# benedikthoward/ENPH459-Super-Resolution

Measured on AMD Instinct MI355X. Metric: HR megapixels/sec at x4 upscale (SAA + 80-iteration IBP reconstruction), higher is better.
Workload: dtype f32; 1 GPU; C2: x4 multi-frame SR of 64x64 LR patches -> 256x256 HR, N=16 frames (all 4x4 sub-pixel phases), 7x7 Gaussian PSF, shift_and_add + ibp(80 it, step 0.5); patches_per_gpu=1024, global_patches=1024, factor=4, frames=16, n_iter=80, parallelism=patch-sharded x1, no collective

## Files before the change

enph459-super-resolution_amd/csrc/srx_api.hip:

```cpp
#include <cstdio>
#include <cstring>

#include "srx_prims.hpp"
#include "srx_fused.hpp"
#include "srx_route.hpp"
#include "srx_btile.hpp"
#include "srx_metrics.hpp"
#include "srx_psf.hpp"
#include "srx_register.hpp"
#include "srx_mean.hpp"
#include "srx_png.hpp"
#include "srx_crc.hpp"
#include "srx_patches.hpp"

using namespace srx;

static thread_local const char *g_last_path = "none";

namespace srx {
Profiler &profiler()
{
    static Profiler p;
    return p;
}
// ... 643 lines not shown
int srx_ibp_plan_get_rows_f32(srx_plan_t *p, int row_lo, int row_hi, float *dst, srx_stream_t s) { return plan_rows<float>(p, row_lo, row_hi, dst, false, hs(s)); }
int srx_ibp_plan_set_rows_f32(srx_plan_t *p, int row_lo, int row_hi, const float *src, srx_stream_t s)
{
    return plan_rows<float>(p, row_lo, row_hi, const_cast<float *>(src), true, hs(s));
}
int srx_ibp_plan_get_rows_f64(srx_plan_t *p, int row_lo, int row_hi, double *dst, srx_stream_t s) { return plan_rows<double>(p, row_lo, row_hi, dst, false, hs(s)); }
int srx_ibp_plan_set_rows_f64(srx_plan_t *p, int row_lo, int row_hi, const double *src, srx_stream_t s)
{
    return plan_rows<double>(p, row_lo, row_hi, const_cast<double *>(src), true, hs(s));
}
const char *srx_ibp_plan_path(srx_plan_t *p) { return p ? p->path : "none"; }
int srx_ibp_plan_supports_trace_rows(srx_plan_t *p) { return p && p->z ? 1 : 0; }
void srx_ibp_plan_destroy(srx_plan_t *p) { delete p; }

int srx_version(void) { return 100; }

#ifdef SRX_STAMPS
int srx_debug_stamps(unsigned long long *host_out)
{
    if (hipDeviceSynchronize() != hipSuccess)
        return SRX_E_HIP;
    if (hipMemcpyFromSymbol(host_out, HIP_SYMBOL(srx::srx_dbg_stamps), sizeof(unsigned long long) * 5 * 8 * 40000) != hipSuccess)
        return SRX_E_HIP;
    return SRX_OK;
}
int srx_debug_pstamps(unsigned long long *host_out)
{
    if (hipDeviceSynchronize() != hipSuccess)
        return SRX_E_HIP;
    if (hipMemcpyFromSymbol(host_out, HIP_SYMBOL(srx::srx_dbg_pstamps), sizeof(unsigned long long) * 24 * 4096) != hipSuccess)
        return SRX_E_HIP;
    return SRX_OK;
}
#endif

const char *srx_strerror(int s)
{
    switch (s) {
    case SRX_OK: return "ok";
    case SRX_E_INVALID: return "invalid argument";
    case SRX_E_UNSUPPORTED: return "unsupported configuration";
    case SRX_E_WORKSPACE: return "workspace missing, not 256-byte aligned or too small";
    case SRX_E_HIP: return "HIP runtime error";
    default: return "unknown status";
    }
}

const char *srx_last_path(void) { return g_last_path; }

void srx_profile_enable(int on)
{
    profiler().clear();
    profiler().on = on != 0;
}

int srx_profile_kernel_count(void) { return KID_COUNT; }

const char *srx_profile_kernel_name(int id) { return id >= 0 && id < KID_COUNT ? g_kernel_names[id] : ""; }

int srx_profile_get(int id, double *total_ms, long *launches)
{
    if (id < 0 || id >= KID_COUNT || !total_ms || !launches)
        return SRX_E_INVALID;
    Profiler &pf = profiler();
    std::lock_guard<std::mutex> g(pf.mu);
    double tot = 0.0;
// ... 416 lines not shown
```

enph459-super-resolution_amd/csrc/srx_common.h:

```cpp
#pragma once
#include <hip/hip_runtime.h>
#include <stddef.h>
#include <stdint.h>
#include <stdlib.h>
#include <string.h>

#include <atomic>
#include <mutex>
#include <type_traits>
#include <vector>

#include "srx.h"

#define SRX_NPAD 12
#define SRX_HORIZON 64

namespace srx {

template <typename T> __host__ __device__ constexpr T pole() { return (T)-0.26794919243112270647; }

template <typename T> struct AxisTap {
    int idx[4];
    T w[4];
};
// ... 254 lines not shown
    const unsigned orig = blockIdx.x + gx * (blockIdx.y + gy * blockIdx.z);
    const unsigned xcd = orig & 7u, q = nwg >> 3, r = nwg & 7u;
    const unsigned id = (xcd < r ? xcd * (q + 1) : r * (q + 1) + (xcd - r) * q) + (orig >> 3);
    bx = (int)(id % gx);
    by = (int)((id / gx) % gy);
    bz = (int)(id / (gx * gy));
}

__device__ __forceinline__ unsigned xcd_index(unsigned orig, unsigned n)
{
    const unsigned xcd = orig & 7u, q = n >> 3, r = n & 7u;
    return (xcd < r ? xcd * (q + 1) : r * (q + 1) + (xcd - r) * q) + (orig >> 3);
}
__device__ __forceinline__ void xcd_block_2d(int &bx, int &by)
{
    const unsigned gx = gridDim.x, id = xcd_index(blockIdx.x + gx * blockIdx.y, gx * gridDim.y);
    bx = (int)(id % gx);
    by = (int)(id / gx);
}

#ifdef SRX_STAMPS
__device__ unsigned long long srx_dbg_stamps[5][8][40000];
#define SRX_STAMP(K, PH)                                                                                       \
    do {                                                                                                        \
        if (threadIdx.x == 0 && threadIdx.y == 0) {                                                             \
            unsigned long long _t;                                                                               \
            asm volatile("s_memtime %0\n\ts_waitcnt lgkmcnt(0)" : "=s"(_t)::"memory");                         \
            const unsigned _blk = blockIdx.x + gridDim.x * (blockIdx.y + gridDim.y * blockIdx.z);                \
            if (_blk < 40000)                                                                                    \
                srx_dbg_stamps[K][PH][_blk] = _t;                                                                \
        }                                                                                                       \
    } while (0)
__device__ unsigned long long srx_dbg_pstamps[24][4096];
#define SRX_PSTAMP(PH)                                                                                         \
    do {                                                                                                        \
        __builtin_amdgcn_sched_barrier(0);                                                                      \
        const unsigned _lb = blockIdx.x + gridDim.x * blockIdx.y;                                               \
        const unsigned _sl = _lb * (blockDim.x >> 6) + (threadIdx.x >> 6);                                      \
        if ((threadIdx.x & 63) == 0 && _sl < 4096 && blockIdx.z == 0) {                                         \
            unsigned long long _t;                                                                               \
            asm volatile("s_memtime %0\n\ts_waitcnt lgkmcnt(0)" : "=s"(_t)::"memory");                         \
            srx_dbg_pstamps[PH][_sl] = _t;                                                                       \
        }                                                                                                       \
        __builtin_amdgcn_sched_barrier(0);                                                                      \
    } while (0)
#else
#define SRX_STAMP(K, PH) do { } while (0)
#define SRX_PSTAMP(PH) do { } while (0)
#endif

__device__ __forceinline__ void err_trace_reduce(const double *__restrict__ epart, int nblk, int item, double base,
                                                 double *__restrict__ out, int tid, double *part4)
{
    const double *p = epart + (size_t)item * nblk;
    double acc[8];
#pragma unroll
    for (int u = 0; u < 8; u++)
        acc[u] = 0.0;
    for (int i = tid; i < nblk; i += 256 * 8) {
#pragma unroll
        for (int u = 0; u < 8; u++) {
            const int k = i + 256 * u;
            acc[u] += k < nblk ? p[k] : 0.0;
        }
    }
    double s = ((acc[0] + acc[1]) + (acc[2] + acc[3])) + ((acc[4] + acc[5]) + (acc[6] + acc[7]));
    s = wave_sum(s);
    if ((tid & 63) == 0)
        part4[tid >> 6] = s;
    __syncthreads();
    if (tid == 0)
        *out = base + ((part4[0] + part4[1]) + (part4[2] + part4[3]));
    __syncthreads();
}

__device__ __forceinline__ void bspline3_weights(double t, double w[4])
{
    double y = t, z = 1.0 - t;
    w[1] = (y * y * (y - 2.0) * 3.0 + 4.0) / 6.0;
    w[2] = (z * z * (z - 2.0) * 3.0 + 4.0) / 6.0;
    w[0] = z * z * z / 6.0;
// ... 5 lines not shown
```

enph459-super-resolution_amd/csrc/srx_mosaic.hpp:

```cpp
#pragma once
#include <algorithm>
#include <type_traits>

#include "srx_fused.hpp"

namespace srx {
namespace mosaic {

constexpr int FWD_BATCH = 24;
using fused::corr7_strip8;
using fused::Kernel7;
using fused::TileCfg;

struct AxisPlan {
    double delta;
    int zero, E, D, PB, RS;
    int n[SRX_MAX_FRAMES];
    int nmin, nmax;
};

struct AxisDev {
    int E, D;
    int n[SRX_MAX_FRAMES];
};

template <typename T> struct MosaicArgs {
    int Dy, Dx, PBy, PBx;
    int RSy, RSx;
    T wfy[4], wfx[4];
    T wby[4], wbx[4];
};

struct MTap {
    int i;
    int rho;
};

static inline bool plan_axis(int N, const double *sh, int axis, int f, AxisPlan &pl)
{
    for (int k = 0; k < N; k++) {
        const double d = sh[2 * k + axis] * f;
        double n = std::floor(d), fr = d - n;
        if (fr > 1.0 - 1e-12)
            n += 1.0, fr = 0.0;
        if (fr < 1e-12)
            fr = 0.0;
        if (k == 0)
            pl.delta = fr;
        else if (std::fabs(fr - pl.delta) > 1e-12)
            return false;
        pl.n[k] = (int)n;
    }
    pl.zero = pl.delta == 0.0;
    pl.E = pl.zero ? 11 : 10;
    pl.D = 13 - pl.E;
    pl.nmin = pl.nmax = pl.n[0];
    for (int k = 1; k < N; k++)
        pl.nmin = std::min(pl.nmin, pl.n[k]), pl.nmax = std::max(pl.nmax, pl.n[k]);
    pl.PB = 13 - pl.nmin;
    pl.RS = std::max(13 - pl.nmax, 0);
    return true;
}

static inline bool eligible(const IbpSpec &s)
{
    if (!fused::ibp_eligible(s) || s.f < 2)
        return false;
    AxisPlan a;
    return plan_axis(s.N, s.sh, 0, s.f, a) && plan_axis(s.N, s.sh, 1, s.f, a) && s.H >= 32 && s.W >= 32;
}

__global__ void __launch_bounds__(64) k_build_mtaps(MTap *__restrict__ tab, int len, int n_img, int f, AxisDev ax)
{
    const int p = blockIdx.x * 64 + threadIdx.x, k = blockIdx.y;
    if (p >= len)
        return;
    const int u = p + ax.n[k] - 13;
    MTap t;
    if (u < 0) {
        t.i = 0;
        t.rho = ax.E - ax.n[k];
    } else if (u <= n_img - 1 && u % f == 0) {
        t.i = u / f;
        t.rho = p - ax.D;
    } else {
        t.i = -1;
        t.rho = 0;
    }
    tab[(size_t)k * len + p] = t;
}

__device__ __forceinline__ int near_index(int p, int q, int Wg, int PBy, int PBx)
{
    return p < PBy ? p * Wg + q : PBy * Wg + (p - PBy) * PBx + q;
}

template <typename T, int IB, int PXT, typename S = T>
__global__ void __launch_bounds__(256)
    k_mosaic_build(const S *__restrict__ lr, int B, int N, int h, int w, const MTap *__restrict__ tabY,
                   const MTap *__restrict__ tabX, int Hg, int Wg, int PBy, int PBx, int Dy, int Dx, int NB,
                   T *__restrict__ Mg, T *__restrict__ Cg, T *__restrict__ Mu, double *__restrict__ Vpart, int tr_lo, int tr_hi)
{
    __shared__ double part[4][IB];
    const int q0 = blockIdx.x * 64 * PXT + threadIdx.x, p = blockIdx.y * 4 + threadIdx.y, b0 = blockIdx.z * IB;
    const int pu = __builtin_amdgcn_readfirstlane(p);
    const size_t item = (size_t)N * h * w;
    double var[IB];
#pragma unroll
    for (int i = 0; i < IB; i++)
        var[i] = 0.0;
    if (pu < Hg) {
        double M[PXT][IB], S1[PXT][IB], S2[PXT][IB];
        int C[PXT], Cu[PXT];
#pragma unroll
        for (int c = 0; c < PXT; c++) {
            C[c] = Cu[c] = 0;
#pragma unroll
            for (int i = 0; i < IB; i++)
                M[c][i] = S1[c][i] = S2[c][i] = 0.0;
        }
        for (int k = 0; k < N; k++) {
            const MTap ty = tabY[(size_t)k * Hg + pu];
// ... 943 lines not shown
{
    return {ar.take<T>(d.B * d.Hg * d.Wg), ar.take<T>(d.Hg * d.Wg), ar.take<T>(d.B * d.NB), ar.take<MTap>(d.N * d.ty), ar.take<MTap>(d.N * d.tx),
            ar.take<double>(d.B), ar.take<double>(d.B * cdiv((int)d.Wg, 64) * cdiv((int)d.Hg, 4)), ar.take<int>(d.NB), ar.take<int>(d.NB * d.NS)};
}
static inline size_t ws_common(const IbpShape &s, int B)
{
    const size_t Hg = s.H + 2 * SRX_NPAD + 3, Wg = s.W + 2 * SRX_NPAD + 3, tl = Hg > Wg ? Hg : Wg;
    const CommonDims d{(size_t)B, (size_t)s.N, Hg, Wg, tl, tl, near_bound(Hg, Wg), near_slots(s.N)};
    return measured([&](Arena &m) { s.eb == 8 ? (void)carve_common<double>(m, d) : (void)carve_common<float>(m, d); });
}

template <typename T, typename S = T>
static int common_prep(Common<T> &c, bool own_build, const IbpCall<T, S> &call, Arena &ar, int tr_lo, int tr_hi)
{
    const IbpSpec &s = call.s;
    const int B = call.B, N = s.N, h = s.h, w = s.w, H = s.H, W = s.W, f = s.f;
    const S *const lr = call.lr;
    const hipStream_t st = call.st;
    const int Hp = H + 2 * SRX_NPAD, Wp = W + 2 * SRX_NPAD, Hg = Hp + 3, Wg = Wp + 3;
    static_assert(std::is_same<S, T>::value || std::is_same<S, uint8_t>::value, "LR samples: T or uint8_t");
    c.lr = lr, c.lr_u8 = !std::is_same<S, T>::value, c.B = B, c.N = N, c.h = h, c.w = w, c.H = H, c.W = W, c.f = f, c.flags = s.flags, c.step = call.step;
    c.scale = 1.0 / ((double)h * (double)w) / (double)N;
    AxisPlan &py = c.py, &px = c.px;
    if (!plan_axis(N, s.sh, 0, f, py) || !plan_axis(N, s.sh, 1, f, px))
        return SRX_E_UNSUPPORTED;
    const int NB = py.PB * Wg + (Hg - py.PB) * px.PB;
    const int NS = (int)near_slots(N);
    c.NB = NB, c.NS = NS, c.Hg = Hg, c.Wg = Wg;
    const auto [Mg, Cg, Mu, tabY, tabX, Vtot, Vpart, ncu, nyx] =
        carve_common<T>(ar, CommonDims{(size_t)B, (size_t)N, (size_t)Hg, (size_t)Wg, (size_t)Hg, (size_t)Wg, (size_t)NB, (size_t)NS});
    if (!ar.ok)
        return SRX_E_WORKSPACE;
    c.Mg = Mg, c.Cg = Cg, c.Mu = Mu, c.tabY = tabY, c.tabX = tabX, c.Vtot = Vtot, c.ncu = ncu, c.nyx = nyx;
    AxisDev dy, dx;
    dy.E = py.E, dy.D = py.D, dx.E = px.E, dx.D = px.D;
    for (int q = 0; q < SRX_MAX_FRAMES; q++)
        dy.n[q] = q < N ? py.n[q] : 0, dx.n[q] = q < N ? px.n[q] : 0;
    MosaicArgs<T> &ma = c.ma;
    ma.Dy = py.D, ma.Dx = px.D, ma.PBy = py.PB, ma.PBx = px.PB, ma.RSy = py.RS, ma.RSx = px.RS;
    fused::axis_firs<T>(py.delta, px.delta, 1.0, ma.wfy, ma.wfx, ma.wby, ma.wbx);
    fused::make_kernel7<T>(s.k, s.kh, s.kw, false, c.kc, s.flags);
    fused::make_kernel7<T>(s.k, s.kh, s.kw, true, c.kt, s.flags);
    c.sep = c.kc.separable && c.kt.separable, c.zero = py.zero && px.zero;
    hipLaunchKernelGGL(k_build_mtaps, dim3(cdiv(Hg, 64), N), dim3(64), 0, st, tabY, Hg, H, f, dy);
    SRX_CHECK_LAUNCH();
    hipLaunchKernelGGL(k_build_mtaps, dim3(cdiv(Wg, 64), N), dim3(64), 0, st, tabX, Wg, W, f, dx);
    SRX_CHECK_LAUNCH();
    if (fill_bytes(Vtot, 0, (size_t)B * sizeof(double), st) != hipSuccess)
        return SRX_E_HIP;
    c.own_build = own_build;
    if (!own_build) {
        if (B >= 8)
            SRX_LAUNCH(KID_MOSAIC_BUILD, (k_mosaic_build<T, 8, 1, S>), dim3(cdiv(Wg, 64), cdiv(Hg, 4), cdiv(B, 8)), dim3(64, 4), 0, st, lr, B, N, h,
                       w, tabY, tabX, Hg, Wg, py.PB, px.PB, py.D, px.D, NB, Mg, Cg, Mu, Vpart, tr_lo, tr_hi);
        else
            SRX_LAUNCH(KID_MOSAIC_BUILD, (k_mosaic_build<T, 1, 4, S>), dim3(cdiv(Wg, 256), cdiv(Hg, 4), B), dim3(64, 4), 0, st, lr, B, N, h, w,
                       tabY, tabX, Hg, Wg, py.PB, px.PB, py.D, px.D, NB, Mg, Cg, Mu, Vpart, tr_lo, tr_hi);
        hipLaunchKernelGGL(k_vtot_reduce, dim3(B), dim3(256), 0, st, Vpart, (B >= 8 ? cdiv(Wg, 64) : cdiv(Wg, 256)) * cdiv(Hg, 4), Vtot);
        SRX_CHECK_LAUNCH();
    }
    hipLaunchKernelGGL(k_build_near, dim3(cdiv(NB, 256)), dim3(256), 0, st, tabY, tabX, N, NS, Hg, Wg, py.PB, px.PB, py.D, px.D,
                       NB, ncu, nyx);
    SRX_CHECK_LAUNCH();
    return SRX_OK;
}

template <typename T> struct TileTabs {
    T *pad, *G;
    double *epart;
};
template <typename T> static TileTabs<T> carve_tiles(Arena &ar, size_t B, int H, int W)
{
    const int Hp = H + 2 * SRX_NPAD, Wp = W + 2 * SRX_NPAD, Hg = Hp + 3, Wg = Wp + 3;
    return {ar.take<T>(B * Hp * Wp), ar.take<T>(B * Hg * Wg), ar.take<double>(B * cdiv(Hg, 32) * cdiv(Wg, 32))};
}
static inline size_t tiles_bytes(const IbpShape &s, int B)
{
    return measured([&](Arena &m) { s.eb == 8 ? (void)carve_tiles<double>(m, B, s.H, s.W) : (void)carve_tiles<float>(m, B, s.H, s.W); });
}

template <typename T>
static int iterate(const Common<T> &c, const T *hr_init, T *hr, int n_iter, double *errors, Arena &ar, hipStream_t st)
{
    const int B = c.B, H = c.H, W = c.W, Hp = H + 2 * SRX_NPAD, Wp = W + 2 * SRX_NPAD, Hg = c.Hg, Wg = c.Wg;
    const auto [pad, G, epart] = carve_tiles<T>(ar, B, H, W);
    if (!ar.ok)
        return SRX_E_WORKSPACE;
    constexpr int TS = TileCfg<T>::T_HR;
#ifdef SRX_ABLATE
    const int dbg = SRX_ABLATE;
#else
    const int dbg = 0;
#endif
// ... 159 lines not shown
```

enph459-super-resolution_amd/csrc/srx_patch.hpp:

```cpp
#pragma once
#include "srx_block.hpp"
#include "srx_mosaic.hpp"

namespace srx {
namespace dtile {
struct AxisTiles {
    int n;
    int o[64], a[65];
};
}
namespace patch {
using namespace blk;
using dtile::AxisTiles;

constexpr int PN = 256;
constexpr int YW = 260;
constexpr int OFF_YT = 16 * RW, OFF_YL = OFF_YT + 4 * YW, OFF_GT = OFF_YL + 4 * YW, OFF_GL = OFF_GT + 3 * YW,
              OFF_ROW = OFF_GL + 3 * YW, OFF_PART = OFF_ROW + PN, LDS_WORDS = OFF_PART + 32;
static_assert(LDS_WORDS * 4 <= 160 * 1024, "LDS budget");

struct AxisW {
    float kb[8];
    float kt[8];
    float wfb[8];
};
struct AxisC {
    int ex;
    int nb;
    int E;
};

constexpr int NN_PAD = 2048;

struct PatchArgs {
    AxisC y, x;
    int nn, ntop;
    int ngrp;
    int c01;
    unsigned long long ry[4], rx[4];
    float sn;
};

struct PatchTabs {
    const float *Mt;
    const unsigned *Mt8;
    const int *m8;
    const float *Ct;
    const AxisW *aw;
    const uint2 *nrec;
    const uint2 *nent;
    const float2 *Mn;
    const float *k2;
// ... 322 lines not shown
    }
#pragma unroll
    for (int m = 0; m < 4; m++) {
        if (test) {
#pragma unroll
            for (int c = 0; c < 4; c++)
                bad |= !((int)(v[m][c] == rintf(v[m][c])) & (int)(v[m][c] >= 0.f) & (int)(v[m][c] <= 255.f));
        }
        tile[cq][wv + 4 * m] = make_float4(v[m][0], v[m][1], v[m][2], v[m][3]);
    }
    if (test) {
        if (__syncthreads_or(bad) && threadIdx.x == 0)
            atomicAnd(&m8[b], 0);
    } else {
        __syncthreads();
    }
    if (bytes) {
#pragma unroll
        for (int n = 0; n < 4; n++) {
            const int u = threadIdx.x + 256 * n, sub = u & 3, r = (u >> 2) & 15, grp = u >> 6, q = 4 * grp + sub;
            const float4 t = tile[q][r];
            const unsigned wd = (unsigned)t.x | (unsigned)t.y << 8 | (unsigned)t.z << 16 | (unsigned)t.w << 24;
            Mt8[(size_t)b * (PN / 4) * PN + ((size_t)grp * PN + gy0 + r) * 4 + sub] = wd;
        }
    } else {
#pragma unroll
        for (int n = 0; n < 4; n++) {
            const int u = threadIdx.x + 256 * n, r = u & 15, q = u >> 4;
            reinterpret_cast<float4 *>(Mt)[((size_t)b * (PN / 4) + q) * PN + gy0 + r] = tile[q][r];
        }
    }
}
template <typename S = float>
__global__ void __launch_bounds__(256)
    k_patch_near_build(const S *__restrict__ lr, int N, int h, int w, const mosaic::MTap *__restrict__ tabY, const mosaic::MTap *__restrict__ tabX,
                       int Hg, int Wg, int Dy, int Dx, int exy, int exx, int nby, int nbx, int nn, float2 *__restrict__ Mn, double *__restrict__ Vtot)
{
    const int t = blockIdx.x * 256 + threadIdx.x, b = blockIdx.y;
    double var = 0.0;
    if (t < nn) {
        int ngy, ngx, dst;
        near_coords(t, PN, exy, exx, nby, nbx, ngy, ngx, dst);
        const int p = ngy + 13, q = ngx + 13;
        const S *src = lr + (size_t)b * N * h * w;
        double M = 0.0, S1 = 0.0, S2 = 0.0;
        int cu = 0;
        for (int k = 0; k < N; k++) {
            const mosaic::MTap ty = tabY[(size_t)k * Hg + p], tx = tabX[(size_t)k * Wg + q];
            if (ty.i < 0 || tx.i < 0)
                continue;
            const double lv = (double)src[((size_t)k * h + ty.i) * w + tx.i];
            M += lv;
            if (ty.rho == p - Dy && tx.rho == q - Dx)
                S1 += lv, S2 += lv * lv, cu++;
        }
        Mn[(size_t)b * NN_PAD + t] = make_float2((float)M, (float)S1);
        if (cu > 1)
            var = S2 - S1 * S1 / (double)cu;
    }
    __shared__ double part[4];
    const double ws = wave_sum(var);
    if ((threadIdx.x & 63) == 0)
        part[threadIdx.x >> 6] = ws;
    __syncthreads();
    if (threadIdx.x == 0) {
        const double sacc = part[0] + part[1] + part[2] + part[3];
        if (sacc != 0.0)
            atomicAdd(&Vtot[b], sacc);
    }
}


struct AxisWPair {
    AxisW y, x;
};

template <bool C01, bool M8, int FORM = 0>
__global__ void __launch_bounds__(1024)
    k_ibp_patch(const float *__restrict__ hr_in, float *__restrict__ hr_out, PatchTabs tb, PatchArgs pa, const double *__restrict__ Vtot,
                double scale, double *__restrict__ errors, int n_iter)
{
    constexpr bool ALL1 = FORM == 1;
    constexpr int PSF = ALL1 ? 0 : FORM;
    static_assert(!ALL1 || (C01 && M8), "the all-ones G step is the byte mosaic's on a full phase grid");
    __shared__ __attribute__((aligned(16))) float lds[LDS_WORDS];
    const int tid0 = threadIdx.x;
    const int wave = __builtin_amdgcn_readfirstlane(tid0 >> 6), s = wave >> 2, u = wave & 3;
    const int b = blockIdx.x;
    float *Rown = lds + wave * RW;
    const float *Rup = lds + (wave - 4) * RW, *Rdn = lds + (wave + 4) * RW;
    const float *Rlf = lds + (wave - 1) * RW, *Rrt = lds + (wave + 1) * RW;
    float *Ystrip = lds + OFF_YT, *Gstrip = lds + OFF_GT, *rowbuf = lds + OFF_ROW;
    float *Yt = lds + OFF_YT, *Yl = lds + OFF_YL, *Gt = lds + OFF_GT, *Gl = lds + OFF_GL;
    double *part = reinterpret_cast<double *>(lds + OFF_PART);
    const int exy = pa.y.ex, exx = pa.x.ex, nby = pa.y.nb, nbx = pa.x.nb;

    const __amdgpu_buffer_rsrc_t rs_in = fused::plane_rsrc(hr_in + (size_t)b * PN * PN, (size_t)PN * PN);
    const __amdgpu_buffer_rsrc_t rs_out = fused::plane_rsrc(hr_out + (size_t)b * PN * PN, (size_t)PN * PN);
    if ((__builtin_amdgcn_readfirstlane(tb.m8[b]) != 0) != M8)
        return;
    constexpr int m8 = M8 ? 1 : 0;
    const float *awy = tb.aw[0].kb, *awx = tb.aw[1].kb;
    const int nn = pa.nn;
    const float sn = pa.sn;
    const int cb0 = (64 * s * PN + 64 * u) * 4;
    const int tb0 = (16 * u * PN + 64 * s) * 16;
    const unsigned long long rmask = C01 ? pa.ry[s] : 0ull, cmask = C01 ? pa.rx[u] : 0ull;

    float a[64];
    {
        const int l4 = (tid0 & 63) * 4;
#pragma unroll
        for (int i = 0; i < 64; i++)
            a[i] = fused::buf_load<float>(rs_in, l4 + (i & 3) * PN * 4, cb0 + (i >> 2) * PN * 16);
    }
    asm volatile("s_waitcnt vmcnt(0)" ::: "memory");
    __syncthreads();
    const int park0 = wave * 16384;
    for (int it = 0; it < n_iter; it++) {
        float r[64];
#define SRX_STAGE_LOCALS()                                 \
    int tid = tid0;                                        \
    asm volatile("" : "+v"(tid));                          \
    const int lane = tid & 63, l4 = lane * 4;              \
    int cbl = cb0, tbl = tb0, m8l = (4 * u * PN + 64 * s) * 16; \
    asm volatile("" : "+s"(cbl), "+s"(tbl), "+s"(m8l));    \
    (void)tbl, (void)m8l, (void)cbl, (void)l4
        float yex = 0.f;
        {
        SRX_STAGE_LOCALS();
        __builtin_amdgcn_sched_barrier(0);
        SRX_PSTAMP(0);
        {
            int pk = park0;
            asm volatile("" : "+s"(pk));
#pragma unroll
            for (int q = 0; q < 16; q++)
                st4(rs_out, l4 * 4, pk + q * 1024, a[4 * q], a[4 * q + 1], a[4 * q + 2], a[4 * q + 3]);
        }
        if (PSF == 0) {
            blur_block(a, s == 0, s == 3, Rown, Rup, Rdn, SLOT0, lane, sload8(awy));
        } else {
            halo3_put(a, Rown, SLOT0, lane);
            __syncthreads();
            const Halo3<float> h = halo3_get(s == 0, s == 3, Rup, Rdn, SLOT0, lane);
            blur2d_cols<PSF == 2 ? 2 : 3>(a, h.lo, h.hi, u == 0, u == 3, Rown, Rlf, Rrt, lane, tb.k2, [](int) {}, [](int, float v) { return v; });
        }
// ... 11 lines not shown
        SRX_PSTAMP(3);
        transpose64(a, r, Rown, lane);
        __builtin_amdgcn_sched_barrier(0);
        SRX_PSTAMP(4);
        }
        float sq = 0.f;
        {
        SRX_STAGE_LOCALS();
        const bool wrapped = exy && s == 3 && lane == 63;
        const int gy = wrapped ? -1 : 64 * s + lane;
        const bool rownear = wrapped || gy < nby;
        const float crow = C01 ? (float)((rmask >> lane) & 1ull) : 0.f;
        if (PSF == 0)
            blur_block(r, u == 0, u == 3, Rown, Rlf, Rrt, SLOT0, lane, sload8(awx));
        __builtin_amdgcn_sched_barrier(0);
        __builtin_amdgcn_sched_barrier(0);
        SRX_PSTAMP(5);
        float yexx = 0.f;
        fwd_chain(r, u == 0, u == 3, Rown, Rlf, Rrt, SLOT1, SLOT0, lane, sload8(awx + 16), yexx);
        __builtin_amdgcn_sched_barrier(0);
        SRX_PSTAMP(6);
        uint2 nr0 = make_uint2(0, 0), nr1 = make_uint2(0, 0), ne0 = make_uint2(0, 0), ne1 = make_uint2(0, 0);
        float2 nm0 = make_float2(0.f, 0.f), nm1 = make_float2(0.f, 0.f);
        const bool n0 = tid < nn, n1 = tid + 1024 < nn;
        const __amdgpu_buffer_rsrc_t rsNr = fused::plane_rsrc(tb.nrec, (size_t)nn), rsNe = fused::plane_rsrc(tb.nent, (size_t)pa.ngrp * NN_PAD),
                                     rsMn = fused::plane_rsrc(tb.Mn + (size_t)b * NN_PAD, (size_t)nn);
        {
            const int t8 = tid * 8;
            nr0 = ld_u2(rsNr, t8), ne0 = ld_u2(rsNe, t8);
            nr1 = ld_u2(rsNr, t8 + 8192), ne1 = ld_u2(rsNe, t8 + 8192);
            const uint2 m0 = ld_u2(rsMn, t8), m1 = ld_u2(rsMn, t8 + 8192);
            nm0 = make_float2(__uint_as_float(m0.x), __uint_as_float(m0.y)), nm1 = make_float2(__uint_as_float(m1.x), __uint_as_float(m1.y));
        }
        near_put_y(r, yexx, wrapped || (s == 0 && lane <= nby), u == 0, gy + exy, u, exx, nbx, Yt, Yl);
        __syncthreads();
        const __amdgpu_buffer_rsrc_t rsM8 = fused::plane_rsrc(tb.Mt8 + (size_t)b * (PN / 4) * PN, (size_t)(PN / 4) * PN);
        unsigned m8w[16];
        if (m8) {
#pragma unroll
            for (int q = 0; q < 4; q++) {
                const u32x4 v = __builtin_amdgcn_raw_buffer_load_b128(rsM8, l4 * 4, m8l + q * PN * 16, 0);
                m8w[4 * q] = v.x, m8w[4 * q + 1] = v.y, m8w[4 * q + 2] = v.z, m8w[4 * q + 3] = v.w;
            }
        }
        __builtin_amdgcn_sched_barrier(0);
        SRX_PSTAMP(7);
        {
            auto px = [&](uint2 nr, uint2 ne, float2 nm, int t) {
                near_px(nr, ne, nm.x, nm.y, Ystrip, Gstrip, [&](int g) { return ld_u2(rsNe, (g * NN_PAD + t) * 8); }, sq);
            };
            if (n0)
                px(nr0, ne0, nm0, tid);
            if (n1)
                px(nr1, ne1, nm1, tid + 1024);
        }
        __syncthreads();
        __builtin_amdgcn_sched_barrier(0);
        SRX_PSTAMP(8);
        float gexx = 0.f;
        {
            const __amdgpu_buffer_rsrc_t rsM = fused::plane_rsrc(tb.Mt + (size_t)b * PN * PN, (size_t)PN * PN);
            const __amdgpu_buffer_rsrc_t rsC = fused::plane_rsrc(tb.Ct, (size_t)PN * PN);
            float sqf = 0.f;
            unsigned long long cm = cmask;
            asm volatile("" : "+s"(cm));
            float gn[3] = {0.f, 0.f, 0.f};
            if (m8) {
                float cq[4] = {0.f, 0.f, 0.f, 0.f};
#pragma unroll
                for (int j = 0; j < 64; j++) {
                    const float mv = (float)((m8w[j >> 2] >> (8 * (j & 3))) & 255u);
                    float g, w;
                    if (C01 && ALL1 && j < 63) {
                        g = mv - r[j];
                        w = 1.f;
                    } else if (C01) {
                        const bool on = (cm >> j) & 1ull;
                        g = on ? fmaf(-crow, r[j], mv) : 0.f;
                        w = 1.f;
                    } else {
                        if ((j & 3) == 0)
                            ld4(rsC, l4 * 4, tbl + (j >> 2) * PN * 16, cq[0], cq[1], cq[2], cq[3]);
                        const float cv = cq[j & 3];
                        g = fmaf(-cv, r[j], mv);
                        w = mosaic::rcp_count(cv);
                    }
                    const float g2 = g * g * w;
                    sqf += g2;
// ... 84 lines not shown
#pragma unroll
                              for (int q = 0; q < 4; q++)
                                  ld4(rs_out, l4 * 4, pk + (4 * bq + q) * 1024, ld[4 * q], ld[4 * q + 1], ld[4 * q + 2], ld[4 * q + 3]);
                          };
                          if (q == 0) {
                              SRX_PSTAMP(13);
                              load16(hv, 0), load16(hw, 1);
                          }
                          if (q == 1)
                              load16(hv, 2);
                          else if (q == 2)
                              load16(hw, 3);
                      };
            auto post = [&](int i, float corr) {
                          return __builtin_amdgcn_fmed3f(fmaf(corr, sn, ((i >> 4) & 1) ? hw[i & 15] : hv[i & 15]), 0.f, 255.f);
                      };
            if (PSF == 0) {
                bwd_chain(r, a, s == 0, s == 3, Rown, Rup, Rdn, SLOT1 + 384, SLOT1, lane, sload8(awy + 16), sload8(awy + 8), nbr.gm1, nbr.gp1, nbr.gp2, gtop, mid, post);
            } else {
                float hl[3], hr[3];
                bwd_chain_x<false>(r, a, s == 0, s == 3, Rown, Rup, Rdn, SLOT1 + 384, SLOT1, lane, sload8(awy + 16), sload8(awy + 8), nbr.gm1, nbr.gp1, nbr.gp2, gtop,
                                   [](int) {}, [](int, float v) { return v; }, hl, hr);
                blur2d_cols<PSF == 2 ? 2 : 3>(a, hl, hr, u == 0, u == 3, Rown, Rlf, Rrt, lane, tb.k2 + 56, mid, post);
            }
        }
        __builtin_amdgcn_sched_barrier(0);
        SRX_PSTAMP(14);
        }
#undef SRX_STAGE_LOCALS
    }
    {
        asm volatile("s_waitcnt vmcnt(0)" ::: "memory");
        __syncthreads();
        const int l4 = (tid0 & 63) * 4;
#pragma unroll
        for (int i = 0; i < 64; i++)
            fused::buf_store<float>(a[i], rs_out, l4 + (i & 3) * PN * 4, cb0 + (i >> 2) * PN * 16);
    }
}

static inline void fill_axis(const mosaic::AxisPlan &pl, const float *cfwd, const float *cbwd, AxisC &ax, AxisW &aw)
{
    const double kq = -6.0 * ZD;
    double wv[4];
    fused::host_weights(1.0 - pl.delta, wv);
    for (int i = 0; i < 4; i++)
        aw.wfb[i] = (float)wv[i];
    fused::host_weights(pl.delta, wv);
    for (int i = 0; i < 4; i++)
        aw.wfb[4 + i] = (float)(kq * wv[i]);
    aw.kb[7] = aw.kt[7] = 0.f;
    for (int i = 0; i < 7; i++)
        aw.kb[i] = (float)(kq * (double)cfwd[i]), aw.kt[i] = cbwd[i];
    ax.ex = pl.nmax, ax.nb = -pl.nmin, ax.E = pl.E;
}
static inline void fill_near(PatchArgs &pa)
{
    pa.ntop = near_top(PN, pa.y.ex, pa.x.ex, pa.y.nb);
    pa.nn = near_count(PN, PN, pa.y.ex, pa.x.ex, pa.y.nb, pa.x.nb);
}

static inline bool c01_masks(const mosaic::AxisPlan &py, const mosaic::AxisPlan &px, int N, int f, unsigned long long ry[4],
                             unsigned long long rx[4])
{
    int ny[SRX_MAX_FRAMES], nx[SRX_MAX_FRAMES], cy = 0, cx = 0;
    for (int k = 0; k < N; k++) {
        bool fy = false, fx = false;
// ... 97 lines not shown
    int *m8;
    float *Ct;
    uint2 *nrec, *nent;
    float2 *Mn;
    AxisW *aw;
    float *k2;
};
static Carved carve(Arena &ar, const Dims &d)
{
    return {ar.take<BuildMaps>(1), ar.take<float>(d.B * PN * PN), ar.take<unsigned>(d.B * (PN / 4) * PN), ar.take<int>(d.B), ar.take<float>((size_t)PN * PN),
            ar.take<uint2>(NN_PAD), ar.take<uint2>(d.ngrp * NN_PAD), ar.take<float2>(d.B * NN_PAD), ar.take<AxisW>(2), ar.take<float>(112)};
}
static inline size_t tabs_bytes(const IbpShape &s, int B)
{
    return measured([&](Arena &m) { carve(m, Dims{(size_t)B, ((size_t)s.N + 3) / 4}); });
}

static int upload_k2(const fused::Kernel7<float> &kc, const fused::Kernel7<float> &kt, float *k2, hipStream_t st)
{
    const double kq = -6.0 * ZD;
    float kv[112];
    for (int c = 0; c < 7; c++)
        for (int r = 0; r < 8; r++) {
            kv[8 * c + r] = r < 7 ? (float)(kq * kq * (double)kc.k[7 * r + c]) : 0.f;
            kv[56 + 8 * c + r] = r < 7 ? kt.k[7 * r + c] : 0.f;
        }
    return upload_record(st, k2, kv);
}

static int iterate(const mosaic::Common<float> &c, const float *hr_init, float *hr, int n_iter, double *errors, Arena &ar, hipStream_t st)
{
    const int B = c.B, N = c.N, f = c.f, NS = c.NS;
    const mosaic::AxisPlan &py = c.py, &px = c.px;
    const int Hg = PN + 27, Wg = PN + 27, ngrp = NS / 4;
    const auto [maps, Mt, Mt8, m8, Ct, nrec, nent, Mn, aw, k2] = carve(ar, Dims{(size_t)B, (size_t)ngrp});
    if (!ar.ok)
        return SRX_E_WORKSPACE;
    PatchArgs pa;
    AxisWPair awp;
    fill_axis(py, c.kc.cy, c.kt.cy, pa.y, awp.y);
    fill_axis(px, c.kc.cx, c.kt.cx, pa.x, awp.x);
    pa.sn = (float)c.step / (float)N;
    fill_near(pa);
    pa.ngrp = ngrp;
    if (pa.nn > NN_PAD)
        return SRX_E_UNSUPPORTED;
    const int gform = gstep_form(py, px, N, f, pa.ry, pa.rx);
    pa.c01 = gform > 0 ? 1 : 0;
    const AxisTiles one = one_region(PN);
    const int nblk = cdiv(pa.nn, 256);
    if (!c.own_build) {
        SRX_TRY((block_setup<float, float2>(c, one, one, PN, PN, pa.y, pa.x, nblk, Mt, Ct, Mt8, m8, nullptr, nrec, nent, Mn, st)));
    } else {
        if (fill_bytes(m8, 0xff, (size_t)B * sizeof(int), st) != hipSuccess)
            return SRX_E_HIP;
        BuildMaps bm;
        int cy[SRX_MAX_FRAMES], cx[SRX_MAX_FRAMES], ny, nx;
        axis_map(py, N, f, bm.y, cy, ny);
        axis_map(px, N, f, bm.x, cx, nx);
        for (int a = 0; a < 4; a++)
            for (int b = 0; b < 4; b++)
                bm.frame[a][b] = 0;
        for (int q = 0; q < N; q++)
            bm.frame[cy[q]][cx[q]] = (signed char)q;
        bm.nby = pa.y.nb, bm.nbx = pa.x.nb;
        SRX_TRY(upload_record(st, maps, bm));
        if (c.lr_u8) {
            if (!(c.flags & SRX_FLAG_DIAG_U8_BYTE_LOADS) && c.w % 4 == 0 && nx * c.w <= PN)
                SRX_LAUNCH(KID_PATCH_BUILD, (k_patch_build<0, uint8_t, true>), dim3(PN / 16, B), dim3(256), 0, st, (const uint8_t *)c.lr, N, c.h, c.w, maps, m8, Mt, Mt8);
            else
                SRX_LAUNCH(KID_PATCH_BUILD, (k_patch_build<0, uint8_t>), dim3(PN / 16, B), dim3(256), 0, st, (const uint8_t *)c.lr, N, c.h, c.w, maps, m8, Mt, Mt8);
        } else {
            SRX_LAUNCH(KID_PATCH_BUILD, k_patch_build<0>, dim3(PN / 16, B), dim3(256), 0, st, (const float *)c.lr, N, c.h, c.w, maps, m8, Mt, Mt8);
            SRX_LAUNCH(KID_PATCH_FLAGS, k_patch_build<1>, dim3(PN / 16, B), dim3(256), 0, st, (const float *)c.lr, N, c.h, c.w, maps, m8, Mt, Mt8);
        }
        if (pa.nn > 0) {
            SRX_TRY(near_tab(c, one, one, PN, PN, pa.y, pa.x, nblk, nullptr, nrec, nent, st));
            if (c.lr_u8)
                hipLaunchKernelGGL(k_patch_near_build<uint8_t>, dim3(nblk, B), dim3(256), 0, st, (const uint8_t *)c.lr, N, c.h, c.w, c.tabY, c.tabX, Hg, Wg, py.D, px.D,
                                   pa.y.ex, pa.x.ex, pa.y.nb, pa.x.nb, pa.nn, Mn, c.Vtot);
            else
                hipLaunchKernelGGL(k_patch_near_build<float>, dim3(nblk, B), dim3(256), 0, st, (const float *)c.lr, N, c.h, c.w, c.tabY, c.tabX, Hg, Wg, py.D, px.D,
                                   pa.y.ex, pa.x.ex, pa.y.nb, pa.x.nb, pa.nn, Mn, c.Vtot);
            SRX_CHECK_LAUNCH();
        }
    }
    SRX_TRY(upload_record(st, aw, awp));
    const int psf = fused::psf_form(c.kc, c.kt);
    if (psf != 0)
        SRX_TRY(upload_k2(c.kc, c.kt, k2, st));
    PatchTabs tb{Mt, Mt8, m8, Ct, aw, nrec, nent, Mn, k2};
#define SRX_PATCH_PAIR(C01_, PSF_)                                                                                                              \
    do {                                                                                                                                        \
        SRX_LAUNCH(KID_IBP_PATCH, (k_ibp_patch<C01_, true, PSF_>), dim3(B), dim3(1024), 0, st, hr_init, hr, tb, pa, c.Vtot, c.scale, errors, n_iter);  \
        SRX_LAUNCH(KID_IBP_PATCH, (k_ibp_patch<C01_, false, PSF_>), dim3(B), dim3(1024), 0, st, hr_init, hr, tb, pa, c.Vtot, c.scale, errors, n_iter); \
    } while (0)
    if (pa.c01) {
        if (psf == 0 && gform == 2) {
            SRX_LAUNCH(KID_IBP_PATCH, (k_ibp_patch<true, true, 1>), dim3(B), dim3(1024), 0, st, hr_init, hr, tb, pa, c.Vtot, c.scale, errors, n_iter);
            SRX_LAUNCH(KID_IBP_PATCH, (k_ibp_patch<true, false, 0>), dim3(B), dim3(1024), 0, st, hr_init, hr, tb, pa, c.Vtot, c.scale, errors, n_iter);
        } else if (psf == 0)
            SRX_PATCH_PAIR(true, 0);
        else if (psf == 2)
            SRX_PATCH_PAIR(true, 2);
        else
            SRX_PATCH_PAIR(true, 3);
    } else {
        if (psf == 0)
            SRX_PATCH_PAIR(false, 0);
        else if (psf == 2)
            SRX_PATCH_PAIR(false, 2);
        else
            SRX_PATCH_PAIR(false, 3);
    }
#undef SRX_PATCH_PAIR
    return SRX_OK;
}
// ... 4 lines not shown
```

Baseline: 5761 HR-MP/s.

## Fuse near-pixel setup into one kernel and stage tail entries in LDS

For the own-build patch path, the MTap table builds, Vtot memset, m8 fill, near_tab and near-build launches are replaced by one k_patch_near_setup kernel. It computes taps inline and writes nrec/nent from an extra block, with per-patch variance reduced in-block instead of via atomics. Inside the IBP patch kernel, the first few spill groups of the near-pixel tails are prefetched into LDS per wave, so the hot loop reads them from LDS instead of global memory. This cuts launch count and per-iteration global loads, but uses more LDS and adds ballot/rank bookkeeping and timing stamps.

New measurement: 5740 HR-MP/s. No clear change (-0.4%).

```diff
diff --git a/enph459-super-resolution_amd/csrc/srx_api.hip b/enph459-super-resolution_amd/csrc/srx_api.hip
--- a/enph459-super-resolution_amd/csrc/srx_api.hip
+++ b/enph459-super-resolution_amd/csrc/srx_api.hip
@@ -699,6 +699,14 @@
         return SRX_E_HIP;
     return SRX_OK;
 }
+int srx_debug_nstamps(unsigned long long *host_out)
+{
+    if (hipDeviceSynchronize() != hipSuccess)
+        return SRX_E_HIP;
+    if (hipMemcpyFromSymbol(host_out, HIP_SYMBOL(srx::srx_dbg_nstamps), sizeof(unsigned long long) * 8 * 4096) != hipSuccess)
+        return SRX_E_HIP;
+    return SRX_OK;
+}
 #endif
 
 const char *srx_strerror(int s)
diff --git a/enph459-super-resolution_amd/csrc/srx_common.h b/enph459-super-resolution_amd/csrc/srx_common.h
--- a/enph459-super-resolution_amd/csrc/srx_common.h
+++ b/enph459-super-resolution_amd/csrc/srx_common.h
@@ -310,7 +310,10 @@
         }                                                                                                       \
     } while (0)
 __device__ unsigned long long srx_dbg_pstamps[24][4096];
-#define SRX_PSTAMP(PH)                                                                                         \
+__device__ unsigned long long srx_dbg_nstamps[8][4096];
+#define SRX_PSTAMP(PH) SRX_WSTAMP(srx_dbg_pstamps, PH)
+#define SRX_NSTAMP(PH) SRX_WSTAMP(srx_dbg_nstamps, PH)
+#define SRX_WSTAMP(ARR, PH)                                                                                    \
     do {                                                                                                        \
         __builtin_amdgcn_sched_barrier(0);                                                                      \
         const unsigned _lb = blockIdx.x + gridDim.x * blockIdx.y;                                               \
@@ -318,13 +321,14 @@
         if ((threadIdx.x & 63) == 0 && _sl < 4096 && blockIdx.z == 0) {                                         \
             unsigned long long _t;                                                                               \
             asm volatile("s_memtime %0\n\ts_waitcnt lgkmcnt(0)" : "=s"(_t)::"memory");                         \
-            srx_dbg_pstamps[PH][_sl] = _t;                                                                       \
+            ARR[PH][_sl] = _t;                                                                                   \
         }                                                                                                       \
         __builtin_amdgcn_sched_barrier(0);                                                                      \
     } while (0)
 #else
 #define SRX_STAMP(K, PH) do { } while (0)
 #define SRX_PSTAMP(PH) do { } while (0)
+#define SRX_NSTAMP(PH) do { } while (0)
 #endif
 
 __device__ __forceinline__ void err_trace_reduce(const double *__restrict__ epart, int nblk, int item, double base,
diff --git a/enph459-super-resolution_amd/csrc/srx_mosaic.hpp b/enph459-super-resolution_amd/csrc/srx_mosaic.hpp
--- a/enph459-super-resolution_amd/csrc/srx_mosaic.hpp
+++ b/enph459-super-resolution_amd/csrc/srx_mosaic.hpp
@@ -35,6 +35,15 @@
     int i;
     int rho;
 };
+
+static inline AxisDev axis_dev(const AxisPlan &pl, int N)
+{
+    AxisDev d;
+    d.E = pl.E, d.D = pl.D;
+    for (int q = 0; q < SRX_MAX_FRAMES; q++)
+        d.n[q] = q < N ? pl.n[q] : 0;
+    return d;
+}
 
 static inline bool plan_axis(int N, const double *sh, int axis, int f, AxisPlan &pl)
 {
@@ -70,24 +79,28 @@
     return plan_axis(s.N, s.sh, 0, s.f, a) && plan_axis(s.N, s.sh, 1, s.f, a) && s.H >= 32 && s.W >= 32;
 }
 
+__device__ __forceinline__ MTap mtap(int p, int n, int n_img, int f, int E, int D)
+{
+    const int u = p + n - 13;
+    MTap t;
+    if (u < 0) {
+        t.i = 0;
+        t.rho = E - n;
+    } else if (u <= n_img - 1 && u % f == 0) {
+        t.i = u / f;
+        t.rho = p - D;
+    } else {
+        t.i = -1;
+        t.rho = 0;
+    }
+    return t;
+}
 __global__ void __launch_bounds__(64) k_build_mtaps(MTap *__restrict__ tab, int len, int n_img, int f, AxisDev ax)
 {
     const int p = blockIdx.x * 64 + threadIdx.x, k = blockIdx.y;
     if (p >= len)
         return;
-    const int u = p + ax.n[k] - 13;
-    MTap t;
-    if (u < 0) {
-        t.i = 0;
-        t.rho = ax.E - ax.n[k];
-    } else if (u <= n_img - 1 && u % f == 0) {
-        t.i = u / f;
-        t.rho = p - ax.D;
-    } else {
-        t.i = -1;
-        t.rho = 0;
-    }
-    tab[(size_t)k * len + p] = t;
+    tab[(size_t)k * len + p] = mtap(p, ax.n[k], n_img, f, ax.E, ax.D);
 }
 
 __device__ __forceinline__ int near_index(int p, int q, int Wg, int PBy, int PBx)
@@ -1097,33 +1110,30 @@
     if (!ar.ok)
         return SRX_E_WORKSPACE;
     c.Mg = Mg, c.Cg = Cg, c.Mu = Mu, c.tabY = tabY, c.tabX = tabX, c.Vtot = Vtot, c.ncu = ncu, c.nyx = nyx;
-    AxisDev dy, dx;
-    dy.E = py.E, dy.D = py.D, dx.E = px.E, dx.D = px.D;
-    for (int q = 0; q < SRX_MAX_FRAMES; q++)
-        dy.n[q] = q < N ? py.n[q] : 0, dx.n[q] = q < N ? px.n[q] : 0;
     MosaicArgs<T> &ma = c.ma;
     ma.Dy = py.D, ma.Dx = px.D, ma.PBy = py.PB, ma.PBx = px.PB, ma.RSy = py.RS, ma.RSx = px.RS;
     fused::axis_firs<T>(py.delta, px.delta, 1.0, ma.wfy, ma.wfx, ma.wby, ma.wbx);
     fused::make_kernel7<T>(s.k, s.kh, s.kw, false, c.kc, s.flags);
     fused::make_kernel7<T>(s.k, s.kh, s.kw, true, c.kt, s.flags);
     c.sep = c.kc.separable && c.kt.separable, c.zero = py.zero && px.zero;
+    c.own_build = own_build;
+    if (own_build)
+        return SRX_OK;
+    const AxisDev dy = axis_dev(py, N), dx = axis_dev(px, N);
     hipLaunchKernelGGL(k_build_mtaps, dim3(cdiv(Hg, 64), N), dim3(64), 0, st, tabY, Hg, H, f, dy);
     SRX_CHECK_LAUNCH();
     hipLaunchKernelGGL(k_build_mtaps, dim3(cdiv(Wg, 64), N), dim3(64), 0, st, tabX, Wg, W, f, dx);
     SRX_CHECK_LAUNCH();
     if (fill_bytes(Vtot, 0, (size_t)B * sizeof(double), st) != hipSuccess)
         return SRX_E_HIP;
-    c.own_build = own_build;
-    if (!own_build) {
-        if (B >= 8)
-            SRX_LAUNCH(KID_MOSAIC_BUILD, (k_mosaic_build<T, 8, 1, S>), dim3(cdiv(Wg, 64), cdiv(Hg, 4), cdiv(B, 8)), dim3(64, 4), 0, st, lr, B, N, h,
-                       w, tabY, tabX, Hg, Wg, py.PB, px.PB, py.D, px.D, NB, Mg, Cg, Mu, Vpart, tr_lo, tr_hi);
-        else
-            SRX_LAUNCH(KID_MOSAIC_BUILD, (k_mosaic_build<T, 1, 4, S>), dim3(cdiv(Wg, 256), cdiv(Hg, 4), B), dim3(64, 4), 0, st, lr, B, N, h, w,
-                       tabY, tabX, Hg, Wg, py.PB, px.PB, py.D, px.D, NB, Mg, Cg, Mu, Vpart, tr_lo, tr_hi);
-        hipLaunchKernelGGL(k_vtot_reduce, dim3(B), dim3(256), 0, st, Vpart, (B >= 8 ? cdiv(Wg, 64) : cdiv(Wg, 256)) * cdiv(Hg, 4), Vtot);
-        SRX_CHECK_LAUNCH();
-    }
+    if (B >= 8)
+        SRX_LAUNCH(KID_MOSAIC_BUILD, (k_mosaic_build<T, 8, 1, S>), dim3(cdiv(Wg, 64), cdiv(Hg, 4), cdiv(B, 8)), dim3(64, 4), 0, st, lr, B, N, h,
+                   w, tabY, tabX, Hg, Wg, py.PB, px.PB, py.D, px.D, NB, Mg, Cg, Mu, Vpart, tr_lo, tr_hi);
+    else
+        SRX_LAUNCH(KID_MOSAIC_BUILD, (k_mosaic_build<T, 1, 4, S>), dim3(cdiv(Wg, 256), cdiv(Hg, 4), B), dim3(64, 4), 0, st, lr, B, N, h, w,
+                   tabY, tabX, Hg, Wg, py.PB, px.PB, py.D, px.D, NB, Mg, Cg, Mu, Vpart, tr_lo, tr_hi);
+    hipLaunchKernelGGL(k_vtot_reduce, dim3(B), dim3(256), 0, st, Vpart, (B >= 8 ? cdiv(Wg, 64) : cdiv(Wg, 256)) * cdiv(Hg, 4), Vtot);
+    SRX_CHECK_LAUNCH();
     hipLaunchKernelGGL(k_build_near, dim3(cdiv(NB, 256)), dim3(256), 0, st, tabY, tabX, N, NS, Hg, Wg, py.PB, px.PB, py.D, px.D,
                        NB, ncu, nyx);
     SRX_CHECK_LAUNCH();
diff --git a/enph459-super-resolution_amd/csrc/srx_patch.hpp b/enph459-super-resolution_amd/csrc/srx_patch.hpp
--- a/enph459-super-resolution_amd/csrc/srx_patch.hpp
+++ b/enph459-super-resolution_amd/csrc/srx_patch.hpp
@@ -16,8 +16,13 @@
 constexpr int PN = 256;
 constexpr int YW = 260;
 constexpr int OFF_YT = 16 * RW, OFF_YL = OFF_YT + 4 * YW, OFF_GT = OFF_YL + 4 * YW, OFF_GL = OFF_GT + 3 * YW,
-              OFF_ROW = OFF_GL + 3 * YW, OFF_PART = OFF_ROW + PN, LDS_WORDS = OFF_PART + 32;
-static_assert(LDS_WORDS * 4 <= 160 * 1024, "LDS budget");
+              OFF_ROW = OFF_GL + 3 * YW, OFF_PART = OFF_ROW + PN, OFF_TAIL = OFF_PART + 32;
+constexpr int TAIL_G = 3, TAIL_PX = 8, LDS_WORDS = OFF_TAIL + 16 * 2 * TAIL_PX * TAIL_G * 2;
+static_assert(LDS_WORDS * 4 <= 160 * 1024 && OFF_TAIL % 2 == 0, "LDS budget");
+__device__ __forceinline__ int lane_rank(unsigned long long mask)
+{
+    return (int)__builtin_amdgcn_mbcnt_hi((unsigned)(mask >> 32), __builtin_amdgcn_mbcnt_lo((unsigned)mask, 0u));
+}
 
 struct AxisW {
     float kb[8];
@@ -406,41 +411,76 @@
     }
 }
 template <typename S = float>
-__global__ void __launch_bounds__(256)
-    k_patch_near_build(const S *__restrict__ lr, int N, int h, int w, const mosaic::MTap *__restrict__ tabY, const mosaic::MTap *__restrict__ tabX,
-                       int Hg, int Wg, int Dy, int Dx, int exy, int exx, int nby, int nbx, int nn, float2 *__restrict__ Mn, double *__restrict__ Vtot)
-{
-    const int t = blockIdx.x * 256 + threadIdx.x, b = blockIdx.y;
-    double var = 0.0;
-    if (t < nn) {
-        int ngy, ngx, dst;
-        near_coords(t, PN, exy, exx, nby, nbx, ngy, ngx, dst);
-        const int p = ngy + 13, q = ngx + 13;
-        const S *src = lr + (size_t)b * N * h * w;
-        double M = 0.0, S1 = 0.0, S2 = 0.0;
-        int cu = 0;
-        for (int k = 0; k < N; k++) {
-            const mosaic::MTap ty = tabY[(size_t)k * Hg + p], tx = tabX[(size_t)k * Wg + q];
-            if (ty.i < 0 || tx.i < 0)
-                continue;
-            const double lv = (double)src[((size_t)k * h + ty.i) * w + tx.i];
-            M += lv;
-            if (ty.rho == p - Dy && tx.rho == q - Dx)
-                S1 += lv, S2 += lv * lv, cu++;
-        }
-        Mn[(size_t)b * NN_PAD + t] = make_float2((float)M, (float)S1);
-        if (cu > 1)
-            var = S2 - S1 * S1 / (double)cu;
-    }
-    __shared__ double part[4];
-    const double ws = wave_sum(var);
-    if ((threadIdx.x & 63) == 0)
-        part[threadIdx.x >> 6] = ws;
+__global__ void __launch_bounds__(1024)
+    k_patch_near_setup(const S *__restrict__ lr, int B, int N, int NS, int h, int w, int f, mosaic::AxisDev dy, mosaic::AxisDev dx, AxisC ay, AxisC ax, int nn,
+                       uint2 *__restrict__ nrec, uint2 *__restrict__ nent, float2 *__restrict__ Mn, double *__restrict__ Vtot, int *__restrict__ m8)
+{
+    __shared__ double part[32];
+    const int b = blockIdx.x, exy = ay.ex, exx = ax.ex, nby = ay.nb, nbx = ax.nb;
+    if (b == B) {
+        for (int t = threadIdx.x; t < nn; t += 1024) {
+            int ngy, ngx, dst;
+            near_coords(t, PN, exy, exx, nby, nbx, ngy, ngx, dst);
+            const int p = ngy + 13, q = ngx + 13;
+            const unsigned long long own = (unsigned long long)strip_off(ngy, ngx, exy, exx, nby);
+            unsigned long long grp = own * 0x0001000100010001ull;
+            int cnt = 0, cu = 0;
+            for (int k = 0; k < N; k++) {
+                const mosaic::MTap ty = mosaic::mtap(p, dy.n[k], PN, f, dy.E, dy.D), tx = mosaic::mtap(q, dx.n[k], PN, f, dx.E, dx.D);
+                if (ty.i < 0 || tx.i < 0)
+                    continue;
+                const int sh = 16 * (cnt & 3);
+                grp = (grp & ~(0xffffull << sh)) | (unsigned long long)strip_off(ty.rho - ay.E, tx.rho - ax.E, exy, exx, nby) << sh;
+                cu += (ty.rho == p - dy.D && tx.rho == q - dx.D) ? 1 : 0;
+                if ((++cnt & 3) == 0) {
+                    nent[(size_t)(cnt / 4 - 1) * NN_PAD + t] = make_uint2((unsigned)grp, (unsigned)(grp >> 32));
+                    grp = own * 0x0001000100010001ull;
+                }
+            }
+            for (int g = cnt / 4; g < NS / 4; g++) {
+                nent[(size_t)g * NN_PAD + t] = make_uint2((unsigned)grp, (unsigned)(grp >> 32));
+                grp = own * 0x0001000100010001ull;
+            }
+            nrec[t] = make_uint2((unsigned)cnt | (unsigned)cu << 8 | (unsigned)dst << 16, (unsigned)own);
+        }
+        return;
+    }
+    if (threadIdx.x == 0)
+        m8[b] = -1;
+    const S *src = lr + (size_t)b * N * h * w;
+#pragma unroll
+    for (int j = 0; j < 2; j++) {
+        const int t = threadIdx.x + 1024 * j;
+        double var = 0.0;
+        if (t < nn) {
+            int ngy, ngx, dst;
+            near_coords(t, PN, exy, exx, nby, nbx, ngy, ngx, dst);
+            const int p = ngy + 13, q = ngx + 13;
+            double M = 0.0, S1 = 0.0, S2 = 0.0;
+            int cu = 0;
+            for (int k = 0; k < N; k++) {
+                const mosaic::MTap ty = mosaic::mtap(p, dy.n[k], PN, f, dy.E, dy.D), tx = mosaic::mtap(q, dx.n[k], PN, f, dx.E, dx.D);
+                if (ty.i < 0 || tx.i < 0)
+                    continue;
+                const double lv = (double)src[((size_t)k * h + ty.i) * w + tx.i];
+                M += lv;
+                if (ty.rho == p - dy.D && tx.rho == q - dx.D)
+                    S1 += lv, S2 += lv * lv, cu++;
+            }
+            Mn[(size_t)b * NN_PAD + t] = make_float2((float)M, (float)S1);
+            if (cu > 1)
+                var = S2 - S1 * S1 / (double)cu;
+        }
+        const double ws = wave_sum(var);
+        if ((threadIdx.x & 63) == 0)
+            part[16 * j + (threadIdx.x >> 6)] = ws;
+    }
     __syncthreads();
     if (threadIdx.x == 0) {
-        const double sacc = part[0] + part[1] + part[2] + part[3];
-        if (sacc != 0.0)
-            atomicAdd(&Vtot[b], sacc);
+        double v = 0.0;
+        for (int c = 0; c < 8; c++)
+            v += part[4 * c] + part[4 * c + 1] + part[4 * c + 2] + part[4 * c + 3];
+        Vtot[b] = v;
     }
 }
 
@@ -457,7 +497,8 @@
     constexpr bool ALL1 = FORM == 1;
     constexpr int PSF = ALL1 ? 0 : FORM;
     static_assert(!ALL1 || (C01 && M8), "the all-ones G step is the byte mosaic's on a full phase grid");
-    __shared__ __attribute__((aligned(16))) float lds[LDS_WORDS];
+    constexpr bool STAGE = C01;
+    __shared__ __attribute__((aligned(16))) float lds[STAGE ? LDS_WORDS : OFF_TAIL];
     const int tid0 = threadIdx.x;
     const int wave = __builtin_amdgcn_readfirstlane(tid0 >> 6), s = wave >> 2, u = wave & 3;
     const int b = blockIdx.x;
@@ -487,6 +528,26 @@
 #pragma unroll
         for (int i = 0; i < 64; i++)
             a[i] = fused::buf_load<float>(rs_in, l4 + (i & 3) * PN * 4, cb0 + (i >> 2) * PN * 16);
+    }
+    auto tail_at = [](unsigned nrx) {
+        const bool tl = (nrx & 255u) > 4u;
+        return tl ? min(lane_rank(__ballot(tl)), TAIL_PX) : TAIL_PX;
+    };
+    if constexpr (STAGE) {
+        const __amdgpu_buffer_rsrc_t rsNr = fused::plane_rsrc(tb.nrec, (size_t)pa.nn), rsNe = fused::plane_rsrc(tb.nent, (size_t)pa.ngrp * NN_PAD);
+        uint2 *tails = reinterpret_cast<uint2 *>(lds + OFF_TAIL) + wave * (2 * TAIL_G * TAIL_PX);
+        const int at0 = tail_at(ld_u2(rsNr, tid0 * 8).x), at1 = tail_at(ld_u2(rsNr, tid0 * 8 + 8192).x);
+        uint2 e0[TAIL_G], e1[TAIL_G];
+#pragma unroll
+        for (int g = 1; g <= TAIL_G; g++)
+            e0[g - 1] = ld_u2(rsNe, (g * NN_PAD + tid0) * 8), e1[g - 1] = ld_u2(rsNe, (g * NN_PAD + tid0 + 1024) * 8);
+#pragma unroll
+        for (int g = 1; g <= TAIL_G; g++) {
+            if (at0 < TAIL_PX && g < pa.ngrp)
+                tails[at0 * TAIL_G + g - 1] = e0[g - 1];
+            if (at1 < TAIL_PX && g < pa.ngrp)
+                tails[(TAIL_PX + at1) * TAIL_G + g - 1] = e1[g - 1];
+        }
     }
     asm volatile("s_waitcnt vmcnt(0)" ::: "memory");
     __syncthreads();
@@ -564,8 +625,17 @@
             const uint2 m0 = ld_u2(rsMn, t8), m1 = ld_u2(rsMn, t8 + 8192);
             nm0 = make_float2(__uint_as_float(m0.x), __uint_as_float(m0.y)), nm1 = make_float2(__uint_as_float(m1.x), __uint_as_float(m1.y));
         }
+#ifdef SRX_STAMPS
+        SRX_NSTAMP(0);
+        near_put_y(r, yexx, wrapped || (s == 0 && lane <= nby), false, gy + exy, u, exx, nbx, Yt, Yl);
+        SRX_NSTAMP(1);
+        near_put_y(r, yexx, false, u == 0, gy + exy, u, exx, nbx, Yt, Yl);
+        SRX_NSTAMP(2);
+#else
         near_put_y(r, yexx, wrapped || (s == 0 && lane <= nby), u == 0, gy + exy, u, exx, nbx, Yt, Yl);
+#endif
         __syncthreads();
+        SRX_NSTAMP(3);
         const __amdgpu_buffer_rsrc_t rsM8 = fused::plane_rsrc(tb.Mt8 + (size_t)b * (PN / 4) * PN, (size_t)(PN / 4) * PN);
         unsigned m8w[16];
         if (m8) {
@@ -578,14 +648,30 @@
         __builtin_amdgcn_sched_barrier(0);
         SRX_PSTAMP(7);
         {
-            auto px = [&](uint2 nr, uint2 ne, float2 nm, int t) {
-                near_px(nr, ne, nm.x, nm.y, Ystrip, Gstrip, [&](int g) { return ld_u2(rsNe, (g * NN_PAD + t) * 8); }, sq);
+            const uint2 *tails = reinterpret_cast<const uint2 *>(lds + (STAGE ? OFF_TAIL : 0)) + wave * (2 * TAIL_G * TAIL_PX);
+#ifdef SRX_STAMPS
+            if (m8)
+                asm volatile("s_waitcnt vmcnt(4)" ::: "memory");
+            else
+                asm volatile("s_waitcnt vmcnt(0)" ::: "memory");
+            SRX_NSTAMP(4);
+#endif
+            auto px = [&](uint2 nr, uint2 ne, float2 nm, int t, const uint2 *tl) {
+                if constexpr (STAGE) {
+                    const int at = tail_at(nr.x);
+                    near_px(nr, ne, nm.x, nm.y, Ystrip, Gstrip, [&](int g) {
+                        return at < TAIL_PX && g <= TAIL_G ? tl[at * TAIL_G + g - 1] : ld_u2(rsNe, (g * NN_PAD + t) * 8);
+                    }, sq);
+                } else {
+                    near_px(nr, ne, nm.x, nm.y, Ystrip, Gstrip, [&](int g) { return ld_u2(rsNe, (g * NN_PAD + t) * 8); }, sq);
+                }
             };
             if (n0)
-                px(nr0, ne0, nm0, tid);
+                px(nr0, ne0, nm0, tid, tails);
             if (n1)
-                px(nr1, ne1, nm1, tid + 1024);
-        }
+                px(nr1, ne1, nm1, tid + 1024, tails + TAIL_G * TAIL_PX);
+        }
+        SRX_NSTAMP(5);
         __syncthreads();
         __builtin_amdgcn_sched_barrier(0);
         SRX_PSTAMP(8);
@@ -736,7 +822,10 @@
     {
         asm volatile("s_waitcnt vmcnt(0)" ::: "memory");
         __syncthreads();
-        const int l4 = (tid0 & 63) * 4;
+        int tid = tid0;
+        if constexpr (STAGE)
+            asm volatile("" : "+v"(tid));
+        const int l4 = (tid & 63) * 4;
 #pragma unroll
         for (int i = 0; i < 64; i++)
             fused::buf_store<float>(a[i], rs_out, l4 + (i & 3) * PN * 4, cb0 + (i >> 2) * PN * 16);
@@ -900,7 +989,7 @@
 {
     const int B = c.B, N = c.N, f = c.f, NS = c.NS;
     const mosaic::AxisPlan &py = c.py, &px = c.px;
-    const int Hg = PN + 27, Wg = PN + 27, ngrp = NS / 4;
+    const int ngrp = NS / 4;
     const auto [maps, Mt, Mt8, m8, Ct, nrec, nent, Mn, aw, k2] = carve(ar, Dims{(size_t)B, (size_t)ngrp});
     if (!ar.ok)
         return SRX_E_WORKSPACE;
@@ -920,8 +1009,14 @@
     if (!c.own_build) {
         SRX_TRY((block_setup<float, float2>(c, one, one, PN, PN, pa.y, pa.x, nblk, Mt, Ct, Mt8, m8, nullptr, nrec, nent, Mn, st)));
     } else {
-        if (fill_bytes(m8, 0xff, (size_t)B * sizeof(int), st) != hipSuccess)
-            return SRX_E_HIP;
+        const mosaic::AxisDev dy = mosaic::axis_dev(py, N), dx = mosaic::axis_dev(px, N);
+        if (c.lr_u8)
+            hipLaunchKernelGGL(k_patch_near_setup<uint8_t>, dim3(B + 1), dim3(1024), 0, st, (const uint8_t *)c.lr, B, N, NS, c.h, c.w, f, dy, dx, pa.y, pa.x, pa.nn,
+                               nrec, nent, Mn, c.Vtot, m8);
+        else
+            hipLaunchKernelGGL(k_patch_near_setup<float>, dim3(B + 1), dim3(1024), 0, st, (const float *)c.lr, B, N, NS, c.h, c.w, f, dy, dx, pa.y, pa.x, pa.nn,
+                               nrec, nent, Mn, c.Vtot, m8);
+        SRX_CHECK_LAUNCH();
         BuildMaps bm;
         int cy[SRX_MAX_FRAMES], cx[SRX_MAX_FRAMES], ny, nx;
         axis_map(py, N, f, bm.y, cy, ny);
@@ -941,16 +1036,6 @@
         } else {
             SRX_LAUNCH(KID_PATCH_BUILD, k_patch_build<0>, dim3(PN / 16, B), dim3(256), 0, st, (const float *)c.lr, N, c.h, c.w, maps, m8, Mt, Mt8);
             SRX_LAUNCH(KID_PATCH_FLAGS, k_patch_build<1>, dim3(PN / 16, B), dim3(256), 0, st, (const float *)c.lr, N, c.h, c.w, maps, m8, Mt, Mt8);
-        }
-        if (pa.nn > 0) {
-            SRX_TRY(near_tab(c, one, one, PN, PN, pa.y, pa.x, nblk, nullptr, nrec, nent, st));
-            if (c.lr_u8)
-                hipLaunchKernelGGL(k_patch_near_build<uint8_t>, dim3(nblk, B), dim3(256), 0, st, (const uint8_t *)c.lr, N, c.h, c.w, c.tabY, c.tabX, Hg, Wg, py.D, px.D,
-                                   pa.y.ex, pa.x.ex, pa.y.nb, pa.x.nb, pa.nn, Mn, c.Vtot);
-            else
-                hipLaunchKernelGGL(k_patch_near_build<float>, dim3(nblk, B), dim3(256), 0, st, (const float *)c.lr, N, c.h, c.w, c.tabY, c.tabX, Hg, Wg, py.D, px.D,
-                                   pa.y.ex, pa.x.ex, pa.y.nb, pa.x.nb, pa.nn, Mn, c.Vtot);
-            SRX_CHECK_LAUNCH();
         }
     }
     SRX_TRY(upload_record(st, aw, awp));
```
